# k-xlsx/huff-encoding

Measured on AMD Instinct MI355X. Metric: encode+decode GB/s on 1 GiB bytes at 1/2/4/8 MI355X; % HBM roofline, higher is better.
Workload: dtype u8; 1 GPU; 1 GiB uniform bytes (BASELINE configs[1]), encode+decode, bit-exact; bytes_per_gpu=1073741824, global_bytes=1073741824, compressed_bytes_per_gpu=1073741824, parallelism=shard1

## Files before the change

huff-encoding_amd/csrc/device/hist.hip:

```cpp
#include "bitreader.hpp"

namespace huff::dev {

namespace {

constexpr int kThreads = 256;
constexpr int kCopies = 32;
#ifndef HUFF_HIST_LOGC
#define HUFF_HIST_LOGC 5
#endif


template <int LOGC = 5>
__device__ __forceinline__ void count_word(uint32_t* h, uint32_t w, uint32_t lane_c) {
#pragma unroll
    for (int k = 0; k < 4; ++k) {
        uint32_t b = (w >> (8 * k)) & 0xFFu;
        __hip_atomic_fetch_add(&h[(b << LOGC) | lane_c], 1u, __ATOMIC_RELAXED, __HIP_MEMORY_SCOPE_WORKGROUP);
    }
}

template <int LOGC = 5>
__device__ __forceinline__ void count_masked(uint32_t* h, uint4 v, uint64_t off, uint64_t lo, uint64_t hi,
                                             uint32_t lane_c) {
    uint32_t w[4] = {v.x, v.y, v.z, v.w};
#pragma unroll
    for (int k = 0; k < 16; ++k) {
        uint64_t g = off + k;
        if (g >= lo && g < hi) {
            uint32_t b = (w[k >> 2] >> (8 * (k & 3))) & 0xFFu;
            __hip_atomic_fetch_add(&h[(b << LOGC) | lane_c], 1u, __ATOMIC_RELAXED, __HIP_MEMORY_SCOPE_WORKGROUP);
        }
    }
}

__global__ __launch_bounds__(kThreads) void k_hist(const uint8_t* __restrict__ base, uint64_t lo, uint64_t hi,
                                                   uint32_t nchunks, uint32_t* __restrict__ chunk_hist,
                                                   unsigned long long* __restrict__ gw) {
    __shared__ __attribute__((aligned(16))) uint32_t h[256 * kCopies];
    const uint32_t t = threadIdx.x;
    const uint32_t lane32 = t & 31;
    for (uint32_t i = t; i < 256 * kCopies; i += kThreads) h[i] = 0;
    uint64_t total = 0;
    __syncthreads();

    for (uint32_t c = blockIdx.x; c < nchunks; c += gridDim.x) {
        const uint64_t cbeg = static_cast<uint64_t>(c) * kChunk;
        const bool full = cbeg >= lo && cbeg + kChunk <= hi;
        if (full) {
            const uint4* p = reinterpret_cast<const uint4*>(base + cbeg) + t;
#pragma unroll 1
            for (int r = 0; r < 16; r += 4) {
                uint4 v0 = ld_nt(p + (r + 0) * kThreads);
                uint4 v1 = ld_nt(p + (r + 1) * kThreads);
                uint4 v2 = ld_nt(p + (r + 2) * kThreads);
                uint4 v3 = ld_nt(p + (r + 3) * kThreads);
                count_word(h, v0.x, lane32); count_word(h, v0.y, lane32);
                count_word(h, v0.z, lane32); count_word(h, v0.w, lane32);
                count_word(h, v1.x, lane32); count_word(h, v1.y, lane32);
                count_word(h, v1.z, lane32); count_word(h, v1.w, lane32);
                count_word(h, v2.x, lane32); count_word(h, v2.y, lane32);
                count_word(h, v2.z, lane32); count_word(h, v2.w, lane32);
                count_word(h, v3.x, lane32); count_word(h, v3.y, lane32);
                count_word(h, v3.z, lane32); count_word(h, v3.w, lane32);
            }
        } else {
            for (int r = 0; r < 16; ++r) {
                const uint64_t off = cbeg + static_cast<uint64_t>(r) * kRound + t * 16;
                if (off + 16 <= lo || off >= hi) continue;
                uint4 v;
                if (off + 16 <= hi) {
                    v = *reinterpret_cast<const uint4*>(base + off);
                } else {
                    uint32_t w[4] = {0, 0, 0, 0};
                    for (int k = 0; off + k < hi; ++k) w[k >> 2] |= static_cast<uint32_t>(base[off + k]) << (8 * (k & 3));
                    v = make_uint4(w[0], w[1], w[2], w[3]);
                }
                count_masked(h, v, off, lo, hi, lane32);
            }
        }
        __syncthreads();
        uint32_t s = 0;
#pragma unroll 8
        for (int j = 0; j < kCopies; ++j) {
            uint32_t k = (j + t) & 31;
            s += h[(t << 5) | k];
            h[(t << 5) | k] = 0;
        }
        if (chunk_hist) chunk_hist[static_cast<uint64_t>(c) * 256 + t] = s;
        total += s;
        __syncthreads();
    }
    if (total) atomicAdd(&gw[(blockIdx.x % kHistCopies) * 256 + t], static_cast<unsigned long long>(total));
}

template <int LOGC>
__global__ __launch_bounds__(512) void k_hist1x2(const uint8_t* __restrict__ base, uint64_t lo, uint64_t hi,
                                                 uint32_t nchunks, uint32_t* __restrict__ chunk_hist,
                                                 unsigned long long* __restrict__ gw) {
    constexpr uint32_t C = 1u << LOGC;
    constexpr int T = 256;
    static_assert(LOGC >= 3 && LOGC <= 6, "k_hist1x2 needs 8..64 LDS copies (64 KiB of static LDS at most)");
    static_assert(kChunk / C < 65536, "a copy's 16-bit half counter must not overflow");
    constexpr int NL = kChunk / 16 / T;
    if (blockIdx.x == 0)
        for (uint32_t i = threadIdx.x; i < kHistCopies * 256 + 1; i += 2 * T) gw[i] = 0;
    __shared__ __attribute__((aligned(16))) uint32_t h[256 * C];
    const uint32_t t = threadIdx.x, tl = t & (T - 1), half = t / T;
    const uint32_t lane_c = t & (C - 1);
    const uint32_t inc = half ? 0x10000u : 1u;
    const uint32_t c = 2 * blockIdx.x + half;
    const uint64_t cbeg = static_cast<uint64_t>(c) * kChunk;
    const bool live = c < nchunks;
    const bool full = live && cbeg >= lo && cbeg + kChunk <= hi;
    uint4 v[NL];
    if (full) {
        const uint4* p = reinterpret_cast<const uint4*>(base + cbeg) + tl;
#pragma unroll
        for (int r = 0; r < NL; ++r) v[r] = ld_nt(p + r * T);
    }
    __builtin_amdgcn_sched_barrier(0);
    uint4* h4 = reinterpret_cast<uint4*>(h);
#pragma unroll
    for (uint32_t i = 0; i < 256 * C / 4 / (2 * T); ++i) h4[t + i * 2 * T] = make_uint4(0, 0, 0, 0);
    __builtin_amdgcn_s_waitcnt(0xc07f);
    __builtin_amdgcn_s_barrier();
    auto add = [&](uint32_t w) {
#pragma unroll
        for (int k = 0; k < 4; ++k)
            __hip_atomic_fetch_add(&h[(((w >> (8 * k)) & 0xFFu) << LOGC) | lane_c], inc, __ATOMIC_RELAXED,
                                   __HIP_MEMORY_SCOPE_WORKGROUP);
    };
    if (full) {
#pragma unroll
        for (int r = 0; r < NL; ++r) {
            add(v[r].x);
            add(v[r].y);
            add(v[r].z);
            add(v[r].w);
        }
    } else if (live) {
        for (int r = 0; r < NL; ++r) {
            const uint64_t off = cbeg + static_cast<uint64_t>(r) * (16 * T) + tl * 16;
            if (off + 16 <= lo || off >= hi) continue;
            for (int k = 0; k < 16; ++k)
                if (off + k >= lo && off + k < hi)
                    __hip_atomic_fetch_add(&h[(static_cast<uint32_t>(base[off + k]) << LOGC) | lane_c], inc,
                                           __ATOMIC_RELAXED, __HIP_MEMORY_SCOPE_WORKGROUP);
        }
    }
    __syncthreads();
    if (t < 256) {
        uint32_t s0 = 0, s1 = 0;
#pragma unroll 8
        for (uint32_t j = 0; j < C; ++j) {
            const uint32_t x = h[(t << LOGC) | ((j + t) & (C - 1))];
            s0 += x & 0xFFFFu;
            s1 += x >> 16;
        }
        chunk_hist[static_cast<uint64_t>(2 * blockIdx.x) * 256 + t] = s0;
        if (2 * blockIdx.x + 1 < nchunks) chunk_hist[static_cast<uint64_t>(2 * blockIdx.x + 1) * 256 + t] = s1;
    }
}

__global__ __launch_bounds__(256) void k_rows_sum(const uint32_t* __restrict__ chunk_hist, uint32_t nchunks,
                                                  unsigned long long* __restrict__ gw) {
    const uint32_t t = threadIdx.x;
    uint64_t s0 = 0, s1 = 0, s2 = 0, s3 = 0;
    uint32_t c = blockIdx.x;
    const uint32_t g = gridDim.x;
    for (; c + 3 * g < nchunks; c += 4 * g) {
        s0 += chunk_hist[static_cast<uint64_t>(c) * 256 + t];
        s1 += chunk_hist[static_cast<uint64_t>(c + g) * 256 + t];
        s2 += chunk_hist[static_cast<uint64_t>(c + 2 * g) * 256 + t];
        s3 += chunk_hist[static_cast<uint64_t>(c + 3 * g) * 256 + t];
    }
    for (; c < nchunks; c += g) s0 += chunk_hist[static_cast<uint64_t>(c) * 256 + t];
    const uint64_t s = s0 + s1 + s2 + s3;
    if (s) atomicAdd(&gw[(blockIdx.x % kHistCopies) * 256 + t], static_cast<unsigned long long>(s));
}

#ifndef HUFF_RP_GROUPS
#define HUFF_RP_GROUPS 128
#endif
constexpr uint32_t kRpWaves = 16;
__global__ __launch_bounds__(kRpWaves * 64) void k_rows_publish(const uint32_t* __restrict__ chunk_hist,
                                                                uint32_t nchunks, unsigned long long* gw,
                                                                unsigned long long* host, uint64_t tag) {
    __shared__ uint64_t part[kRpWaves][256];
    __shared__ uint32_t last;
    const uint32_t t = threadIdx.x, lane = t & 63, wave = t >> 6;
    const uint32_t stride = gridDim.x * kRpWaves;
    const uint4* rows = reinterpret_cast<const uint4*>(chunk_hist) + lane;
    uint64_t a0 = 0, a1 = 0, a2 = 0, a3 = 0;
    uint32_t c = blockIdx.x * kRpWaves + wave;
    for (; c + 3 * stride < nchunks; c += 4 * stride) {
        uint4 v[4];
#pragma unroll
        for (int k = 0; k < 4; ++k) v[k] = rows[static_cast<uint64_t>(c + k * stride) * 64];
#pragma unroll
        for (int k = 0; k < 4; ++k) {
            a0 += v[k].x;
            a1 += v[k].y;
            a2 += v[k].z;
            a3 += v[k].w;
        }
    }
    for (; c < nchunks; c += stride) {
        const uint4 v = rows[static_cast<uint64_t>(c) * 64];
        a0 += v.x;
        a1 += v.y;
        a2 += v.z;
        a3 += v.w;
    }
    part[wave][4 * lane] = a0;
    part[wave][4 * lane + 1] = a1;
    part[wave][4 * lane + 2] = a2;
    part[wave][4 * lane + 3] = a3;
    __syncthreads();
    if (t < 256) {
        uint64_t s = 0;
#pragma unroll
        for (uint32_t w = 0; w < kRpWaves; ++w) s += part[w][t];
        if (s)
            __hip_atomic_fetch_add(&gw[(blockIdx.x % kHistCopies) * 256 + t], static_cast<unsigned long long>(s),
                                   __ATOMIC_RELAXED, __HIP_MEMORY_SCOPE_AGENT);
    }
    __syncthreads();
    if (t == 0) {
        const unsigned long long k = __hip_atomic_fetch_add(&gw[kHistCopies * 256], 1ull, __ATOMIC_ACQ_REL,
                                                            __HIP_MEMORY_SCOPE_AGENT);
        last = k == gridDim.x - 1u;
    }
    __syncthreads();
    if (!last || t >= 256) return;
    __atomic_thread_fence(__ATOMIC_ACQUIRE);
    uint64_t tot = 0;
#pragma unroll
    for (uint32_t k = 0; k < kHistCopies; ++k)
        tot += __hip_atomic_load(&gw[k * 256 + t], __ATOMIC_RELAXED, __HIP_MEMORY_SCOPE_AGENT);
    __hip_atomic_store(&host[t], (tag << 48) | tot, __ATOMIC_RELAXED, __HIP_MEMORY_SCOPE_SYSTEM);
}

__global__ __launch_bounds__(256) void k_hist_row(const unsigned long long* __restrict__ gw,
                                                  const uint8_t* __restrict__ in, uint64_t n,
                                                  long long* __restrict__ row) {
    const uint32_t t = threadIdx.x;
    uint64_t tot = 0;
#pragma unroll
    for (uint32_t k = 0; k < kHistCopies; ++k) tot += gw[k * 256 + t];
    row[t] = static_cast<long long>(tot);
    if (t == 0) {
        const uint32_t m = n < 8 ? static_cast<uint32_t>(n) : 8u;
        uint64_t packed = 0;
        for (uint32_t i = 0; i < m; ++i) packed |= static_cast<uint64_t>(in[n - m + i]) << (8 * i);
        row[256] = static_cast<long long>(packed);
        row[257] = m;
    }
}

__global__ __launch_bounds__(256) void k_chunk_bits(const uint32_t* __restrict__ chunk_hist, uint32_t nchunks,
                                                    CodeLens lens, uint64_t* __restrict__ bits) {
    const uint8_t* len = lens.len;
    const uint32_t wave = threadIdx.x >> 6, lane = threadIdx.x & 63;
    const uint32_t c = blockIdx.x * 4 + wave;
    if (c >= nchunks) return;
    uint4 hv = reinterpret_cast<const uint4*>(chunk_hist + static_cast<uint64_t>(c) * 256)[lane];
    uint32_t lv = reinterpret_cast<const uint32_t*>(len)[lane];
    uint64_t s = static_cast<uint64_t>(hv.x) * (lv & 0xFF) + static_cast<uint64_t>(hv.y) * ((lv >> 8) & 0xFF) +
                 static_cast<uint64_t>(hv.z) * ((lv >> 16) & 0xFF) + static_cast<uint64_t>(hv.w) * (lv >> 24);
#pragma unroll
    for (int d = 32; d >= 1; d >>= 1) s += __shfl_down(s, d, 64);
    if (lane == 0) bits[c] = s;
}

__global__ __launch_bounds__(1024) void k_scan_tiles(const uint64_t* __restrict__ bits, uint32_t nchunks,
                                                     uint64_t* __restrict__ start, uint64_t* __restrict__ tsum) {
    __shared__ uint32_t wsum[16];
    const uint32_t t = threadIdx.x, lane = t & 63, wave = t >> 6;
    const uint32_t i = blockIdx.x * 1024 + t;
    const uint32_t v = i < nchunks ? static_cast<uint32_t>(bits[i]) : 0u;
    const uint32_t incl = wave_scan_incl(v);
    if (lane == 63) wsum[wave] = incl;
    __syncthreads();
    uint32_t pre = 0, tot = 0;
#pragma unroll
    for (uint32_t w = 0; w < 16; ++w) {
        pre += (w < wave) ? wsum[w] : 0u;
        tot += wsum[w];
    }
    if (i < nchunks) start[i] = pre + incl - v;
    if (t == 0) tsum[blockIdx.x] = tot;
}

__global__ __launch_bounds__(1024) void k_scan_tsum(uint32_t tiles, uint64_t* __restrict__ tsum) {
    __shared__ uint64_t wsum[16];
    const uint32_t t = threadIdx.x, lane = t & 63, wave = t >> 6;
    const uint32_t per = (tiles + 1023) / 1024;
    const uint32_t lo = t * per < tiles ? t * per : tiles, hi = lo + per < tiles ? lo + per : tiles;
    uint64_t mine = 0;
    for (uint32_t q = lo; q < hi; ++q) mine += tsum[q];
    uint64_t incl = mine;
#pragma unroll
    for (int d = 1; d < 64; d <<= 1) {
        const uint64_t v = __shfl_up(incl, d, 64);
        if (lane >= static_cast<uint32_t>(d)) incl += v;
    }
    if (lane == 63) wsum[wave] = incl;
    __syncthreads();
    uint64_t pre = 0, tot = 0;
#pragma unroll
    for (uint32_t w = 0; w < 16; ++w) {
        pre += (w < wave) ? wsum[w] : 0u;
        tot += wsum[w];
    }
    uint64_t run = pre + incl - mine;
    for (uint32_t q = lo; q < hi; ++q) {
        const uint64_t v = tsum[q];
        tsum[q] = run;
        run += v;
    }
    if (t == 0) tsum[tiles] = tot;
}

__device__ __forceinline__ void publish_total(unsigned long long* host, uint64_t tag, uint64_t total) {
    if (host) __hip_atomic_store(host, (tag << 48) | total, __ATOMIC_RELAXED, __HIP_MEMORY_SCOPE_SYSTEM);
}

__global__ __launch_bounds__(1024) void k_scan_fix_small(uint32_t nchunks, uint64_t base,
                                                         const uint64_t* __restrict__ tsum,
                                                         uint64_t* __restrict__ start,
                                                         unsigned long long* host, uint64_t tag) {
    __shared__ uint64_t off;
    const uint32_t t = threadIdx.x;
    if (t < 64) {
        uint64_t sum = t < blockIdx.x ? tsum[t] : 0;
#pragma unroll
        for (int d = 32; d >= 1; d >>= 1) sum += __shfl_down(sum, d, 64);
        if (t == 0) off = base + sum;
    }
    __syncthreads();
    const uint32_t i = blockIdx.x * 1024 + t;
    if (i < nchunks) start[i] += off;
    if (blockIdx.x == gridDim.x - 1 && t == 0) {
        const uint64_t end = off + tsum[blockIdx.x];
        start[nchunks] = end;
        publish_total(host, tag, end - base);
    }
}

__global__ __launch_bounds__(1024) void k_scan_fix(uint32_t nchunks, uint64_t base, const uint64_t* __restrict__ tsum,
                                                   uint64_t* __restrict__ start, unsigned long long* host,
                                                   uint64_t tag) {
    const uint32_t t = threadIdx.x;
    const uint64_t off = base + tsum[blockIdx.x];
    const uint32_t i = blockIdx.x * 1024 + t;
    if (i < nchunks) start[i] += off;
    if (blockIdx.x == gridDim.x - 1 && t == 0) {
        start[nchunks] = base + tsum[gridDim.x];
        publish_total(host, tag, tsum[gridDim.x]);
    }
}

__global__ __launch_bounds__(256) void k_find_first(const uint8_t* __restrict__ in, uint64_t n,
                                                    const uint8_t* __restrict__ mask,
                                                    unsigned long long* __restrict__ pos) {
    __shared__ uint8_t m[256];
    m[threadIdx.x] = mask[threadIdx.x];
    __syncthreads();
    for (uint64_t i = static_cast<uint64_t>(blockIdx.x) * blockDim.x + threadIdx.x; i < n;
         i += static_cast<uint64_t>(gridDim.x) * blockDim.x) {
        if (m[in[i]]) {
            atomicMin(pos, static_cast<unsigned long long>(i));
            return;
        }
    }
}

}

hipError_t launch_hist(const uint8_t* base, uint64_t lo, uint64_t hi, uint32_t nchunks, uint32_t* chunk_hist,
                       unsigned long long* gw, hipStream_t s, HistDone done) {
    if (nchunks == 0) return hipSuccess;
    if (chunk_hist) {
        launch_k(k_hist1x2<HUFF_HIST_LOGC>, dim3((nchunks + 1) / 2), dim3(512), 0, s, base, lo, hi, nchunks,
                           chunk_hist, gw);
        if (done.host) {
            const uint32_t want = (nchunks + 4 * kRpWaves - 1) / (4 * kRpWaves);
            const uint32_t g = want < HUFF_RP_GROUPS ? want : HUFF_RP_GROUPS;
            launch_k(k_rows_publish, dim3(g), dim3(kRpWaves * 64), 0, s, chunk_hist, nchunks, gw, done.host,
                     done.tag);
            return hipGetLastError();
        }
        const uint32_t g = nchunks < 512 ? nchunks : 512;
        launch_k(k_rows_sum, dim3(g), dim3(256), 0, s, chunk_hist, nchunks, gw);
        return hipGetLastError();
    }
    uint32_t grid = nchunks < 1024 ? nchunks : 1024;
    const hipError_t e = hipMemsetAsync(gw, 0, kHistCopies * 256 * 8, s);
    if (e != hipSuccess) return e;
    launch_k(k_hist, dim3(grid), dim3(kThreads), 0, s, base, lo, hi, nchunks, chunk_hist, gw);
    return hipGetLastError();
}

hipError_t launch_hist_row(const unsigned long long* gw, const uint8_t* in, uint64_t n, long long* row,
                           hipStream_t s) {
    launch_k(k_hist_row, dim3(1), dim3(256), 0, s, gw, in, n, row);
    return hipGetLastError();
}

hipError_t launch_chunk_bits(const uint32_t* chunk_hist, uint32_t nchunks, const CodeLens& len, uint64_t* bits,
                             hipStream_t s) {
    if (nchunks == 0) return hipSuccess;
    launch_k(k_chunk_bits, dim3((nchunks + 3) / 4), dim3(256), 0, s, chunk_hist, nchunks, len, bits);
    return hipGetLastError();
}

hipError_t launch_scan(const uint64_t* bits, uint32_t nchunks, uint64_t base, uint64_t* start, uint64_t* tsum,
                       hipStream_t s, HistDone done) {
    const uint32_t tiles = nchunks ? (nchunks + 1023) / 1024 : 1;
    launch_k(k_scan_tiles, dim3(tiles), dim3(1024), 0, s, bits, nchunks, start, tsum);
    if (tiles <= 64) {
        launch_k(k_scan_fix_small, dim3(tiles), dim3(1024), 0, s, nchunks, base, tsum, start, done.host,
                           done.tag);
    } else {
        launch_k(k_scan_tsum, dim3(1), dim3(1024), 0, s, tiles, tsum);
        launch_k(k_scan_fix, dim3(tiles), dim3(1024), 0, s, nchunks, base, tsum, start, done.host,
                           done.tag);
    }
    return hipGetLastError();
}

hipError_t launch_find_first(const uint8_t* in, uint64_t n, const uint8_t* missing_mask, unsigned long long* pos,
                             hipStream_t s) {
    if (n == 0) return hipSuccess;
    uint64_t blocks = (n + 255) / 256;
    uint32_t grid = blocks < 4096 ? static_cast<uint32_t>(blocks) : 4096;
    launch_k(k_find_first, dim3(grid), dim3(256), 0, s, in, n, missing_mask, pos);
    return hipGetLastError();
}

}
```

huff-encoding_amd/csrc/device/kernels.hpp:

```cpp
#pragma once

#include <hip/hip_runtime.h>
#ifdef __HIPCC__
#include <hip/hip_ext.h>
#endif

#include <cstdint>

namespace huff::dev {

struct LaunchEvents {
    hipEvent_t start = nullptr, stop = nullptr;
};
LaunchEvents& launch_events();
#ifdef __HIPCC__
template <typename F, typename... Args>
inline void launch_k(F kernel, dim3 grid, dim3 block, uint32_t lds, hipStream_t s, Args... args) {
    LaunchEvents& e = launch_events();
    if (e.stop) {
        hipExtLaunchKernelGGL(kernel, grid, block, lds, s, e.start, e.stop, 0, args...);
        e.start = nullptr;
    } else {
        hipLaunchKernelGGL(kernel, grid, block, lds, s, args...);
    }
// ... 333 lines not shown
    const uint8_t* blobs;
    const uint64_t* payload_begin;
    const uint64_t* comp_off;
    const uint32_t* status;
    uint32_t nstreams;
    uint8_t* comp;
    uint64_t comp_cap;
};
struct BatchCountArgs {
    const uint8_t* comp;
    const uint64_t* comp_off;
    const uint64_t* bits;
    const uint64_t* codes;
    const uint32_t* status_in;
    uint32_t nstreams;
    uint64_t* seg;
    uint64_t seg_cap;
    uint64_t* counts;
    uint32_t* status;
};
struct BatchIndexArgs {
    const uint8_t* comp;
    const uint64_t* comp_off;
    const uint64_t* bits;
    const uint64_t* codes;
    const uint64_t* seg;
    uint64_t seg_cap;
    const uint64_t* off;
    const uint64_t* idx_off;
    uint32_t* status;
    uint32_t nstreams;
    uint32_t* sub;
    uint64_t sub_cap;
};
hipError_t launch_batch_blob_offsets(const BatchBlobArgs& a, hipStream_t s);
hipError_t launch_batch_to_bytes(const BatchBlobArgs& a, hipStream_t s);
hipError_t launch_batch_parse(const BatchParseArgs& a, hipStream_t s);
hipError_t launch_batch_unwrap(const BatchUnwrapArgs& a, hipStream_t s);
hipError_t launch_batch_count(const BatchCountArgs& a, hipStream_t s);
hipError_t launch_batch_index(const BatchIndexArgs& a, hipStream_t s);

constexpr uint32_t kDeepWords = 8;
struct DeepPackArgs;
struct DeepSerialArgs {
    const uint8_t* comp;
    uint64_t comp_bytes;
    uint64_t valid_bits;
    const uint32_t* lut;
    uint32_t lut_bits;
    uint8_t* out;
    uint64_t cap;
    unsigned long long* count;
    unsigned long long* end;
};
struct WalkEndArgs {
    const uint8_t* comp;
    uint64_t comp_bytes;
    const uint32_t* lut;
    uint32_t lut_bits;
    const uint64_t* start;
    uint64_t start_v;
    uint32_t start_packed;
    const uint64_t* count;
    uint64_t count_v;
    unsigned long long* end;
};
hipError_t launch_walk_end(const WalkEndArgs& a, hipStream_t s);
hipError_t launch_shift_bits(const uint8_t* src, uint8_t* dst, uint64_t n, uint32_t r, hipStream_t s);
hipError_t launch_pack_deep(const DeepPackArgs& a, hipStream_t s);
hipError_t launch_decode_deep(const DecodeArgs& a, hipStream_t s);
hipError_t launch_decode_deep_serial(const DeepSerialArgs& a, hipStream_t s);

size_t pack_lds_bytes(bool long_codes, uint32_t max_len, uint32_t stage_words);
uint32_t pack_round_bytes();
uint32_t pack_waves_per_group(bool long_codes);
uint32_t pack_groups_per_cu(bool long_codes, uint32_t max_len, size_t lds);
size_t decode_lds_bytes(uint32_t lut_bits);
constexpr uint32_t kDecodeFixed = 10;
constexpr uint32_t kDecodeFixedCheck = 11;

struct HistDone {
    unsigned long long* host = nullptr;
    uint64_t tag = 0;
};
hipError_t launch_hist(const uint8_t* base, uint64_t lo, uint64_t hi, uint32_t nchunks, uint32_t* chunk_hist,
                       unsigned long long* gw, hipStream_t s, HistDone done = HistDone{});
hipError_t launch_hist_row(const unsigned long long* gw, const uint8_t* in, uint64_t n, long long* row,
                           hipStream_t s);
struct alignas(8) CodeLens {
    uint8_t len[256];
};
struct DeepPackArgs {
    CodeLens len;
    const uint32_t* words;
    const uint8_t* in;
    uint64_t n;
    const uint64_t* chunk_start;
    uint32_t nchunks;
    uint8_t* out;
    uint32_t* sub_bit;
};
hipError_t launch_chunk_bits(const uint32_t* chunk_hist, uint32_t nchunks, const CodeLens& len, uint64_t* bits,
                             hipStream_t s);
hipError_t launch_scan(const uint64_t* bits, uint32_t nchunks, uint64_t base, uint64_t* start, uint64_t* tsum,
                       hipStream_t s, HistDone done = HistDone{});
hipError_t launch_pack(bool long_codes, const PackArgs& a, hipStream_t s);
hipError_t launch_decode(const DecodeArgs& a, hipStream_t s);
hipError_t launch_decode_fixed(const DecodeArgs& a, hipStream_t s);
uint32_t decode_fixed_builds();
const char* decode_fixed_build_name(uint32_t i);
uint64_t decode_fixed_build_launches(uint32_t i);
uint32_t decode_fixed_index_forms();
const char* decode_fixed_index_form_name(uint32_t i);
uint64_t decode_fixed_index_form_launches(uint32_t i);
struct RangeReq {
    uint64_t first, count, out_begin, piece0;
    uint32_t index;
    uint32_t pad;
};
struct RangesArgs {
    const uint8_t* comp;
    uint64_t comp_bytes;
    const uint32_t* lut;
    uint32_t lut_bits;
    const uint64_t* chunk_start;
    const uint32_t* sub_bit;
    const uint16_t* sub16;
    const uint64_t* task_base;
    uint32_t nchunks;
    uint64_t n;
    const RangeReq* req;
    uint32_t nreq;
    uint64_t npieces;
    uint8_t* out;
    uint32_t* status;
};
hipError_t launch_decode_ranges(const RangesArgs& a, hipStream_t s);
uint32_t decode_ranges_index_forms();
const char* decode_ranges_index_form_name(uint32_t i);
uint64_t decode_ranges_index_form_launches(uint32_t i);
hipError_t launch_indexless_spec(const IndexlessArgs& a, hipStream_t s);
hipError_t launch_indexless_settle_all(const IndexlessArgs& a, hipStream_t s);
hipError_t launch_indexless_emit(const IndexlessArgs& a, const uint64_t* off, uint8_t* out, hipStream_t s);
hipError_t launch_indexless_counts(const IndexlessArgs& a, hipStream_t s);
constexpr uint32_t mark32_skip(uint32_t m) { return m & 0x3FFu; }
constexpr uint32_t mark32_rel(uint32_t m) { return (m >> 10) & 0x7FFu; }
constexpr uint32_t mark32_seg(uint32_t m, uint32_t base_seg) { return base_seg + (((m >> 21) - base_seg) & 0x7FFu); }
hipError_t launch_indexless_mark_lite(const IndexlessArgs& a, const uint64_t* off, const unsigned long long* woff,
                                      uint64_t* sub_abs, uint64_t sub_cap, hipStream_t st,
                                      uint32_t* mark32 = nullptr, uint32_t* task_seg = nullptr);
constexpr uint64_t kSkipPosMask = (1ull << 48) - 1;
hipError_t launch_indexless_mark(const IndexlessArgs& a, const uint64_t* off, uint64_t* sub_abs, uint32_t shift,
                                 hipStream_t s);
bool indexless_staged(const IndexlessArgs& a);
hipError_t launch_bytemap(const BytemapArgs& a, hipStream_t s);
hipError_t launch_task_sums(const uint8_t* x, uint64_t n, uint64_t* sums, hipStream_t s);
hipError_t launch_task_sums_check(const uint8_t* x, uint64_t n, const uint64_t* sums, unsigned int* err,
                                  hipStream_t s);
hipError_t launch_find_first(const uint8_t* in, uint64_t n, const uint8_t* missing_mask, unsigned long long* pos,
                             hipStream_t s);
hipError_t launch_generate(int kind, uint64_t seed, uint64_t offset, const uint64_t* cdf, uint8_t* out, uint64_t n,
                           hipStream_t s);
hipError_t launch_calib(int mode, const uint8_t* src, uint8_t* dst, uint64_t n, unsigned* sink, uint32_t cu_count,
                        hipStream_t s);

}
```

huff-encoding_amd/csrc/runtime/runtime.cpp:

```cpp
#include "runtime.hpp"

#include "../host/range_plan.hpp"

#include <algorithm>
#include <cctype>
#include <chrono>
#include <cstdio>
#include <cstdlib>
#include <cstring>
#include <string>
#include <thread>

namespace {

std::atomic<uint64_t> g_tree_ids{1};

}

static_assert(huff::kLutPtr == huff::dev::kLutPtr, "host/dectables.hpp mirrors dev::kLutPtr");
static_assert(huff::kLutMaxBits == huff::dev::kLutMaxBits, "host/dectables.hpp mirrors dev::kLutMaxBits");
static_assert(huff::kSsMaxBits == huff::dev::kSsMaxBits, "host/dectables.hpp mirrors dev::kSsMaxBits");
static_assert(huff::kSsSlow == huff::dev::kSsSlow, "host/dectables.hpp mirrors dev::kSsSlow");
static_assert(huff::kLongMaxLen == huff::dev::kLongMaxLen, "host/dectables.hpp mirrors dev::kLongMaxLen");

// ... 176 lines not shown
        return huff::Status::ok();
    }
    hipEvent_t ev[2];
    for (auto& e : ev) {
        if (!free_events.empty()) {
            e = free_events.back();
            free_events.pop_back();
        } else {
            static const unsigned flags = [] {
                const char* f = std::getenv("HUFF_TIME_FENCE");
                if (f && !std::strcmp(f, "none")) return unsigned(hipEventDisableSystemFence);
                if (f && !std::strcmp(f, "device")) return unsigned(hipEventReleaseToDevice);
                return 0u;
            }();
            HIP_TRY(hipEventCreateWithFlags(&e, flags));
        }
    }
    static const bool markers = [] {
        const char* m = std::getenv("HUFF_TIME_MARKERS");
        return m && *m == '1';
    }();
    auto& le = huff::dev::launch_events();
    if (markers) HIP_TRY(hipEventRecord(ev[0], stream));
    else le = {ev[0], ev[1]};
    const hipError_t err = launch();
    const bool none = le.start != nullptr;
    le = {};
    HIP_TRY(err);
    if (none && !markers) HIP_TRY(hipEventRecord(ev[0], stream));
    if (none || markers) HIP_TRY(hipEventRecord(ev[1], stream));
    pending.push_back({name, ev[0], ev[1]});
    return huff::Status::ok();
}

huff::Status huff_ctx::collect_timing() {
    if (pending.empty()) return huff::Status::ok();
    HIP_TRY(hipStreamSynchronize(stream));
    for (auto& p : pending) {
        float ms = 0.f;
        HIP_TRY(hipEventElapsedTime(&ms, p.a, p.b));
        auto& k = kstats[p.name];
        k.first += ms;
        k.second += 1;
        free_events.push_back(p.a);
        free_events.push_back(p.b);
    }
    pending.clear();
    return huff::Status::ok();
}

huff::Status huff_ctx::sync() {
    HIP_TRY(hipStreamSynchronize(stream));
    return huff::Status::ok();
}

huff::Status huff_ctx::upload_dec_tables(const huff_tree* t, const huff::DecTables** dt, bool for_decode) {
    HUFF_TRY(t->dec_tables(dt));
    if (lut_tree_id == t->id) return huff::Status::ok();
    if (for_decode && (*dt)->all8 && !huff::fixed8_disabled()) return huff::Status::ok();
    const size_t bytes = (*dt)->lut.size() * 4;
    HUFF_TRY(pin_lut.ensure(bytes));
    std::memcpy(pin_lut.p, (*dt)->lut.data(), bytes);
    HUFF_TRY(d_lut.ensure(bytes));
    HIP_TRY(hipStreamWaitEvent(copy_stream, lut_free, 0));
    HIP_TRY(hipMemcpyAsync(d_lut.p, pin_lut.p, bytes, hipMemcpyHostToDevice, copy_stream));
    HIP_TRY(hipEventRecord(pin_lut.ev, copy_stream));
    HIP_TRY(hipStreamWaitEvent(stream, pin_lut.ev, 0));
    lut_tree_id = t->id;
    return huff::Status::ok();
}

huff::Status huff_enc::init(huff_ctx* c, const uint8_t* d, uint64_t nbytes) {
    if (reinterpret_cast<uintptr_t>(d) & 15)
        return huff::Status::err(HUFF_E_INVALID_ARG, "device input must be 16-byte aligned");
    if (nbytes >= (1ull << 48))
        return huff::Status::err(HUFF_E_INVALID_ARG, "one job holds fewer than 2^48 bytes");
    ctx = c;
    d_in = d;
    n = nbytes;
    nchunks = static_cast<uint32_t>((n + huff::dev::kChunk - 1) / huff::dev::kChunk);
    have_hist = packed = sums_valid = false;
    const size_t nc = std::max<uint32_t>(nchunks, 1);
    HUFF_TRY(chunk_hist.ensure(nc * 256 * 4));
    HUFF_TRY(gw.ensure(huff::dev::kHistCopies * 256 * 8 + 8));

    HUFF_TRY(chunk_bits.ensure(nc * 8));
    HUFF_TRY(chunk_start.ensure((nc + 1) * 8));
    HUFF_TRY(tsum.ensure((nc / 1024 + 2) * 8));
    HUFF_TRY(sub_bit.ensure(((n + huff::dev::kIdx - 1) / huff::dev::kIdx + 1) * 4));
    HUFF_TRY(mask.ensure(256));
    HUFF_TRY(pos.ensure(8));
    return huff::Status::ok();
}

class SpinWait {
public:
    bool check_due() {
        if ((++spin_ & 255) != 0) return false;
        const auto now = std::chrono::steady_clock::now();
        if (now - t0_ < std::chrono::milliseconds(2)) return false;
        std::this_thread::yield();
        if (now - last_ < std::chrono::milliseconds(1)) return false;
        last_ = now;
        return true;
    }

private:
    std::chrono::steady_clock::time_point t0_ = std::chrono::steady_clock::now(), last_{};
    uint64_t spin_ = 0;
};

huff::Status TaggedWords::arm(size_t words, huff::dev::HistDone* done) {
    HUFF_TRY(pin.ensure(words * 8));
    if (!dev) {
        std::memset(pin.p, 0, words * 8);
        HIP_TRY(hipHostGetDevicePointer(&dev, pin.p, 0));
    }
    seq = (seq % 0xFFFF) + 1;
    done->host = static_cast<unsigned long long*>(dev);
    done->tag = seq;
    return huff::Status::ok();
}

huff::Status TaggedWords::wait(hipStream_t s, uint64_t tag, uint64_t* out, size_t words, const char* what) {
    const uint64_t* hw = static_cast<const uint64_t*>(pin.p);
    size_t b = 0;
    SpinWait sw;
    while (b < words) {
        const uint64_t v = __atomic_load_n(&hw[b], __ATOMIC_ACQUIRE);
        if ((v >> 48) == tag) {
            out[b++] = v & ((1ull << 48) - 1);
            continue;
        }
        if (sw.check_due()) {
            const hipError_t q = hipStreamQuery(s);
            if (q == hipSuccess && (__atomic_load_n(&hw[b], __ATOMIC_ACQUIRE) >> 48) != tag)
                return huff::Status::err(HUFF_E_HIP, what);
            if (q != hipSuccess && q != hipErrorNotReady) HIP_TRY(q);
        }
    }
    return huff::Status::ok();
}

huff::Status huff_enc::launch_publish(uint64_t* tag) {
    huff::dev::HistDone done;
    HUFF_TRY(ctx->weights.arm(256, &done));
    HUFF_TRY(ctx->timed("hist", [&] {
        return huff::dev::launch_hist(d_in, 0, n, nchunks, static_cast<uint32_t*>(chunk_hist.p),
                                      static_cast<unsigned long long*>(gw.p), ctx->stream, done);
    }));
    *tag = done.tag;
    return huff::Status::ok();
}

static huff::Status pending_guard(const huff_ctx* ctx, const huff_enc* e) {
    if (ctx->hist_pending && ctx->hist_pending != e)
        return huff::Status::err(HUFF_E_STATE, "another job's pass 1 is pending on this context (huff_enc_hist_launch): "
                                               "compress or hist that job first");
    return huff::Status::ok();
}

huff::Status huff_enc::hist_launch() {
    HUFF_TRY(ctx->activate());
    HUFF_TRY(pending_guard(ctx, this));
    if (nchunks == 0 || ctx->hist_pending == this) return huff::Status::ok();
    uint64_t tag = 0;
    HUFF_TRY(launch_publish(&tag));
    ctx->hist_pending = this;
    ctx->hist_pending_tag = tag;
    return huff::Status::ok();
}

huff::Status huff_enc::hist() {
    HUFF_TRY(ctx->activate());
    HUFF_TRY(pending_guard(ctx, this));
    if (nchunks == 0) {
        for (int b = 0; b < 256; ++b) w[b] = 0;
        have_hist = true;
        packed = false;
        return huff::Status::ok();
    }
    uint64_t tag = 0;
    if (ctx->hist_pending == this) {
        tag = ctx->hist_pending_tag;
        ctx->hist_pending = nullptr;
    } else {
        HUFF_TRY(launch_publish(&tag));
    }
    HUFF_TRY(ctx->weights.wait(ctx->stream, tag, w, 256, "pass 1 finished without publishing its weights"));
    have_hist = true;
    packed = false;
    return huff::Status::ok();
}

huff::Status huff_enc::hist_known(const uint64_t counts[256]) {
    HUFF_TRY(ctx->activate());
    if (ctx->hist_pending == this) ctx->hist_pending = nullptr;
    std::memcpy(w, counts, sizeof w);
    have_hist = true;
    packed = false;
    if (nchunks == 0) return huff::Status::ok();
    return ctx->timed("hist", [&] {
        return huff::dev::launch_hist(d_in, 0, n, nchunks, static_cast<uint32_t*>(chunk_hist.p),
                                      static_cast<unsigned long long*>(gw.p), ctx->stream);
    });
}

huff::Status huff_enc::hist_row(long long* d_row) {
    HUFF_TRY(ctx->activate());
    if (ctx->hist_pending == this) ctx->hist_pending = nullptr;
    hipStream_t s = ctx->stream;
    have_hist = false;
    if (nchunks == 0) {
        HIP_TRY(hipMemsetAsync(d_row, 0, 258 * 8, s));
        return huff::Status::ok();
    }
    HUFF_TRY(ctx->timed("hist", [&] {
        hipError_t e = huff::dev::launch_hist(d_in, 0, n, nchunks, static_cast<uint32_t*>(chunk_hist.p),
                                              static_cast<unsigned long long*>(gw.p), s);
        if (e != hipSuccess) return e;
        return huff::dev::launch_hist_row(static_cast<const unsigned long long*>(gw.p), d_in, n, d_row, s);
    }));
    return huff::Status::ok();
}

huff::Status huff_enc::bits(const huff_tree* t, uint64_t* total) {
    if (!have_hist) return huff::Status::err(HUFF_E_STATE, "huff_enc_hist must run before bits/pack");
    const huff::EncTables& et = t->enc_tables();
    uint64_t b = 0;
    for (int i = 0; i < 256; ++i) {
        if (w[i] && et.len[i] == 0) {
            uint8_t m[256];
            for (int k = 0; k < 256; ++k) m[k] = (w[k] && et.len[k] == 0) ? 1 : 0;
            HUFF_TRY(ctx->activate());
            HIP_TRY(hipMemcpy(mask.p, m, 256, hipMemcpyHostToDevice));
            unsigned long long init = ~0ull;
            HIP_TRY(hipMemcpy(pos.p, &init, 8, hipMemcpyHostToDevice));
            HIP_TRY(huff::dev::launch_find_first(d_in, n, static_cast<const uint8_t*>(mask.p),
                                                 static_cast<unsigned long long*>(pos.p), ctx->stream));
            unsigned long long p = 0;
            HIP_TRY(hipMemcpyAsync(&p, pos.p, 8, hipMemcpyDeviceToHost, ctx->stream));
            HUFF_TRY(ctx->sync());
            uint8_t letter = 0;
            HIP_TRY(hipMemcpy(&letter, d_in + p, 1, hipMemcpyDeviceToHost));
            huff::Status st = huff::Status::err(HUFF_E_MISSING_LETTER, "letter not found in codes");
            st.missing_letter = letter;
            return st;
        }
        b += w[i] * et.len[i];
    }
    *total = b;
    return huff::Status::ok();
}

huff::Status huff_enc::check_sums(const uint8_t* d_out) {
    if (!sums_valid || !huff::decode_check_mode()) return huff::Status::ok();
    HUFF_TRY(ctx->d_err.ensure(32));
    unsigned int* err = static_cast<unsigned int*>(ctx->d_err.p);
    const unsigned int init[2] = {0u, ~0u};
    HIP_TRY(hipMemcpyAsync(err, init, 8, hipMemcpyHostToDevice, ctx->stream));
    HIP_TRY(huff::dev::launch_task_sums_check(d_out, n, static_cast<const uint64_t*>(task_sums.p), err, ctx->stream));
    unsigned int e[2] = {};
    HIP_TRY(hipMemcpyAsync(e, err, 8, hipMemcpyDeviceToHost, ctx->stream));
    HUFF_TRY(ctx->sync());
    if (e[0] == 0) return huff::Status::ok();
    return huff::Status::err(HUFF_E_CORRUPT, "decode self-check: letter checksums differ in " + std::to_string(e[0]) +
                                                 " task(s) of 4096 letters; first: task " + std::to_string(e[1]));
}

huff::PackStamps& huff::pack_stamps() {
    static thread_local PackStamps p;
    return p;
}

huff::Status huff_enc::pack(const huff_tree* t, uint64_t base, const uint8_t* prev_tail, size_t prev_tail_len,
                            uint8_t* d_out, size_t out_cap, uint64_t* total) {
    auto& ps = huff::pack_stamps();
    ps.bits = ps.launch = ps.launched = {};
    uint64_t tb = 0;
    HUFF_TRY(bits(t, &tb));
    ps.bits = std::chrono::steady_clock::now();
    compact_index = false;
    const uint64_t need = ((base & 7) + tb + 7) / 8;
    if (total) *total = tb;
    if (need > out_cap) return huff::Status::err(HUFF_E_BUFFER_TOO_SMALL, "output buffer too small");
    if (prev_tail_len > 8) return huff::Status::err(HUFF_E_INVALID_ARG, "prev_tail holds at most 8 bytes");
    HUFF_TRY(ctx->activate());
    hipStream_t s = ctx->stream;
    sums_valid = false;
    if (huff::decode_check_mode() && n) {
        HUFF_TRY(task_sums.ensure(((n + huff::dev::kTaskSym - 1) / huff::dev::kTaskSym) * 8));
        HIP_TRY(huff::dev::launch_task_sums(d_in, n, static_cast<uint64_t*>(task_sums.p), s));
        sums_valid = true;
    }
    const huff::EncTables& et = t->enc_tables();
    const bool long_codes = et.maxlen > huff::dev::kShortMaxLen;
    if ((base & 7) == 0 && et.maxlen == 8 && !huff::fixed8_disabled()) {
        bool all8 = true;
        for (int b = 0; b < 256; ++b) all8 &= (w[b] == 0 || et.len[b] == 8);
        if (all8) {
            huff::dev::BytemapArgs m{};
            m.src = d_in;
            m.dst = d_out;
            m.n = n;
            for (int b = 0; b < 256; ++b) m.map[b] = static_cast<uint8_t>(et.code[b]);
            m.nchunks = nchunks;
// ... 785 lines not shown
```

huff-encoding_amd/csrc/runtime/runtime.hpp:

```cpp
#pragma once

#include <hip/hip_runtime.h>

#include <atomic>
#include <chrono>
#include <functional>
#include <map>
#include <memory>
#include <mutex>
#include <string>
#include <vector>

#include "../device/kernels.hpp"
#include "../host/dectables.hpp"
#include "../host/huff_coding.hpp"

namespace huff {

inline Status hip_status(hipError_t e, const char* what) {
    if (e == hipSuccess) return Status::ok();
    return Status::err(HUFF_E_HIP, std::string(what) + ": " + hipGetErrorString(e));
}
#define HIP_TRY_RT(expr) HUFF_TRY(::huff::hip_status((expr), #expr))

// ... 76 lines not shown
namespace huff {
struct IndexlessSync;
struct FileWs;
}

struct huff_wenc;

struct huff_ctx {
    int device = 0;
    int cu_count = 256;
    hipStream_t own = nullptr;
    hipStream_t stream = nullptr;
    hipStream_t copy_stream = nullptr;
    hipEvent_t lut_free = nullptr;
    TaggedWords weights;
    const huff_enc* hist_pending = nullptr;
    uint64_t hist_pending_tag = 0;
    TaggedWords total;
    PinnedBuf pin_lut;
    DevBuf d_in, d_out;
    DevBuf d_lut;
    const uint16_t* lut_u16(uint32_t off) const {
        return reinterpret_cast<const uint16_t*>(static_cast<const uint32_t*>(d_lut.p) + off);
    }
    DevBuf d_align;
    DevBuf d_comp_align;
    DevBuf d_err;
    std::shared_ptr<huff::IndexlessSync> idx_ws;
    DevBuf idx_sub_abs;
    DevBuf idx_mark32, idx_task_seg;
    huff::IndexlessSync& indexless_ws();
    std::shared_ptr<huff::FileWs> file_ws;
    std::shared_ptr<huff_wenc> wdec_ws;
    uint64_t lut_tree_id = 0;

    struct Timed {
        std::string name;
        hipEvent_t a, b;
    };
    bool timing = false;
    std::vector<Timed> pending;
    std::vector<hipEvent_t> free_events;
    std::map<std::string, std::pair<double, uint64_t>> kstats;
    huff::Status timed(const char* name, const std::function<hipError_t()>& launch);
    huff::Status collect_timing();

    huff::Status activate() const;
    huff::Status upload_dec_tables(const huff_tree* t, const huff::DecTables** dt, bool for_decode = false);
    huff::Status sync();
};

struct huff_enc {
    huff_ctx* ctx = nullptr;
    const uint8_t* d_in = nullptr;
    uint64_t n = 0;
    uint32_t nchunks = 0;
    DevBuf chunk_hist, gw, chunk_bits, chunk_start, tsum, sub_bit, mask, pos;
    DevBuf deep_words;
    DevBuf task_base, sub16;
    bool compact_index = false;
    DevBuf task_sums;
    bool sums_valid = false;
    huff::Status check_sums(const uint8_t* d_out);
    huff::Status expand_index();
    uint64_t w[256] = {};
    bool have_hist = false;
    bool packed = false;
    uint64_t packed_tree_id = 0;
    uint8_t packed_len[256] = {};
    uint64_t packed_code[256] = {};
    std::vector<uint32_t> packed_deep;
    bool packed_any_tree = false;
    void remember_tree(const huff_tree* t);
    bool codes_match(const huff_tree* t) const;
    uint64_t bit_base = 0, total_bits = 0;
    bool index_pending = false;
    huff::Status ensure_index();
    void set_packed(const huff_tree* t, uint64_t base, uint64_t bits, bool pending, bool compact);

    huff::Status init(huff_ctx* c, const uint8_t* d, uint64_t nbytes);
    huff::Status hist();
    huff::Status hist_launch();
    huff::Status launch_publish(uint64_t* tag);
    huff::Status hist_known(const uint64_t counts[256]);
    huff::Status hist_row(long long* d_row);
    huff::Status bits(const huff_tree* t, uint64_t* total);
    huff::Status pack(const huff_tree* t, uint64_t bit_base, const uint8_t* prev_tail, size_t prev_tail_len,
                      uint8_t* d_out, size_t out_cap, uint64_t* total);
    huff::Status decode(const huff_tree* t, const uint8_t* d_comp, uint64_t comp_bytes, uint8_t* d_out);
    DevBuf range_req, range_status;
    huff::Status decode_ranges(const huff_tree* t, const uint8_t* d_comp, uint64_t comp_bytes, const uint64_t* first,
                               const uint64_t* count, const uint64_t* out_begin, uint32_t nreq, uint8_t* d_out,
                               size_t out_cap, uint32_t* status);
    huff::Status download_index(huff_index_host& idx);
    huff::Status upload_index(const huff_index_host& idx);
};

namespace huff {
Status weights_from_host(huff_ctx* ctx, const uint8_t* bytes, size_t n, ByteWeights& out);
Status weights_threaded_from_host(huff_ctx* ctx, const uint8_t* bytes, size_t n, size_t thread_num,
                                  ByteWeights& out);
Status compress_host(huff_ctx* ctx, const uint8_t* bytes, size_t n, const huff_tree* t, huff_compress_data** out);
Status decompress_host(huff_ctx* ctx, const huff_compress_data* cd, uint8_t* out, size_t cap, size_t* out_len);
Status decompress_range_host(huff_ctx* ctx, const huff_compress_data* cd, uint64_t first, uint64_t count,
                             uint8_t* out, size_t cap);
Status file_compress(huff_ctx* ctx, const char* src, const char* dst, size_t block_size);
Status file_decompress(huff_ctx* ctx, const char* src, const char* dst, size_t block_size);
Status parse_block_size(const char* s, size_t* out);
Status run_checked_decode(huff_ctx* ctx, dev::DecodeArgs& a, const std::function<hipError_t()>& launch);
Status decode_indexless_dev(huff_ctx* ctx, const uint8_t* d_comp, uint64_t comp_bytes, uint64_t valid_bits,
                            const huff_tree* t, DevBuf& out, uint64_t* nsym, uint8_t* d_user = nullptr,
                            size_t user_cap = 0, unsigned long long* d_end = nullptr);
struct IndexlessSync {
    const DecTables* dt = nullptr;
    DevBuf s, x0, c, off, flag, tsum, samp, tm, dl, fixlist, chain, rec;
    DevBuf wtot, woff;
    dev::IndexlessArgs a{};
    uint64_t total = 0;
    bool block_off = false;
};
Status indexless_sync(huff_ctx* ctx, const uint8_t* d_comp, uint64_t comp_bytes, uint64_t valid_bits,
                      const huff_tree* t, IndexlessSync& st, bool need_off = true,
                      const std::function<Status()>& before_wait = nullptr);
Status indexless_mark(huff_ctx* ctx, IndexlessSync& st, DevBuf& sub_abs, uint32_t shift = 8);
Status decode_indexless_host(huff_ctx* ctx, const uint8_t* comp, size_t len, uint64_t valid_bits,
                             const huff_tree* t, std::vector<uint8_t>& out);
}
```

Before: 1243 GB/s.

## Fuse histogram row reduction and publish into the pass-1 histogram kernel

```diff
diff --git a/huff-encoding_amd/csrc/device/hist.hip b/huff-encoding_amd/csrc/device/hist.hip
--- a/huff-encoding_amd/csrc/device/hist.hip
+++ b/huff-encoding_amd/csrc/device/hist.hip
@@ -97,14 +97,12 @@
 template <int LOGC>
 __global__ __launch_bounds__(512) void k_hist1x2(const uint8_t* __restrict__ base, uint64_t lo, uint64_t hi,
                                                  uint32_t nchunks, uint32_t* __restrict__ chunk_hist,
-                                                 unsigned long long* __restrict__ gw) {
+                                                 unsigned long long* bins, uint32_t parts, HistDone done) {
     constexpr uint32_t C = 1u << LOGC;
     constexpr int T = 256;
     static_assert(LOGC >= 3 && LOGC <= 6, "k_hist1x2 needs 8..64 LDS copies (64 KiB of static LDS at most)");
     static_assert(kChunk / C < 65536, "a copy's 16-bit half counter must not overflow");
     constexpr int NL = kChunk / 16 / T;
-    if (blockIdx.x == 0)
-        for (uint32_t i = threadIdx.x; i < kHistCopies * 256 + 1; i += 2 * T) gw[i] = 0;
     __shared__ __attribute__((aligned(16))) uint32_t h[256 * C];
     const uint32_t t = threadIdx.x, tl = t & (T - 1), half = t / T;
     const uint32_t lane_c = t & (C - 1);
@@ -150,6 +148,7 @@
         }
     }
     __syncthreads();
+    const bool publish = done.host || done.row;
     if (t < 256) {
         uint32_t s0 = 0, s1 = 0;
 #pragma unroll 8
@@ -160,102 +159,38 @@
         }
         chunk_hist[static_cast<uint64_t>(2 * blockIdx.x) * 256 + t] = s0;
         if (2 * blockIdx.x + 1 < nchunks) chunk_hist[static_cast<uint64_t>(2 * blockIdx.x + 1) * 256 + t] = s1;
-    }
-}
-
-__global__ __launch_bounds__(256) void k_rows_sum(const uint32_t* __restrict__ chunk_hist, uint32_t nchunks,
-                                                  unsigned long long* __restrict__ gw) {
-    const uint32_t t = threadIdx.x;
-    uint64_t s0 = 0, s1 = 0, s2 = 0, s3 = 0;
-    uint32_t c = blockIdx.x;
-    const uint32_t g = gridDim.x;
-    for (; c + 3 * g < nchunks; c += 4 * g) {
-        s0 += chunk_hist[static_cast<uint64_t>(c) * 256 + t];
-        s1 += chunk_hist[static_cast<uint64_t>(c + g) * 256 + t];
-        s2 += chunk_hist[static_cast<uint64_t>(c + 2 * g) * 256 + t];
-        s3 += chunk_hist[static_cast<uint64_t>(c + 3 * g) * 256 + t];
-    }
-    for (; c < nchunks; c += g) s0 += chunk_hist[static_cast<uint64_t>(c) * 256 + t];
-    const uint64_t s = s0 + s1 + s2 + s3;
-    if (s) atomicAdd(&gw[(blockIdx.x % kHistCopies) * 256 + t], static_cast<unsigned long long>(s));
-}
-
-#ifndef HUFF_RP_GROUPS
-#define HUFF_RP_GROUPS 128
-#endif
-constexpr uint32_t kRpWaves = 16;
-__global__ __launch_bounds__(kRpWaves * 64) void k_rows_publish(const uint32_t* __restrict__ chunk_hist,
-                                                                uint32_t nchunks, unsigned long long* gw,
-                                                                unsigned long long* host, uint64_t tag) {
-    __shared__ uint64_t part[kRpWaves][256];
-    __shared__ uint32_t last;
-    const uint32_t t = threadIdx.x, lane = t & 63, wave = t >> 6;
-    const uint32_t stride = gridDim.x * kRpWaves;
-    const uint4* rows = reinterpret_cast<const uint4*>(chunk_hist) + lane;
-    uint64_t a0 = 0, a1 = 0, a2 = 0, a3 = 0;
-    uint32_t c = blockIdx.x * kRpWaves + wave;
-    for (; c + 3 * stride < nchunks; c += 4 * stride) {
-        uint4 v[4];
-#pragma unroll
-        for (int k = 0; k < 4; ++k) v[k] = rows[static_cast<uint64_t>(c + k * stride) * 64];
-#pragma unroll
-        for (int k = 0; k < 4; ++k) {
-            a0 += v[k].x;
-            a1 += v[k].y;
-            a2 += v[k].z;
-            a3 += v[k].w;
-        }
-    }
-    for (; c < nchunks; c += stride) {
-        const uint4 v = rows[static_cast<uint64_t>(c) * 64];
-        a0 += v.x;
-        a1 += v.y;
-        a2 += v.z;
-        a3 += v.w;
-    }
-    part[wave][4 * lane] = a0;
-    part[wave][4 * lane + 1] = a1;
-    part[wave][4 * lane + 2] = a2;
-    part[wave][4 * lane + 3] = a3;
-    __syncthreads();
-    if (t < 256) {
-        uint64_t s = 0;
-#pragma unroll
-        for (uint32_t w = 0; w < kRpWaves; ++w) s += part[w][t];
-        if (s)
-            __hip_atomic_fetch_add(&gw[(blockIdx.x % kHistCopies) * 256 + t], static_cast<unsigned long long>(s),
-                                   __ATOMIC_RELAXED, __HIP_MEMORY_SCOPE_AGENT);
-    }
-    __syncthreads();
-    if (t == 0) {
-        const unsigned long long k = __hip_atomic_fetch_add(&gw[kHistCopies * 256], 1ull, __ATOMIC_ACQ_REL,
+        if (publish) {
+            constexpr uint64_t kSum = (1ull << kHistCntShift) - 1;
+            const uint32_t p = blockIdx.x % parts;
+            const uint32_t adders = (gridDim.x - p + parts - 1) / parts;
+            unsigned long long* word = bins + 256 + p * 256 + t;
+            const uint32_t s = s0 + s1;
+            const uint64_t was = __hip_atomic_fetch_add(word, (1ull << kHistCntShift) | s, __ATOMIC_RELAXED,
+                                                        __HIP_MEMORY_SCOPE_AGENT);
+            if ((was >> kHistCntShift) + 1 == adders) {
+                __hip_atomic_store(word, 0ull, __ATOMIC_RELAXED, __HIP_MEMORY_SCOPE_AGENT);
+                const uint64_t rowsum = (was & kSum) + s;
+                const uint64_t bin = __hip_atomic_fetch_add(&bins[t], (1ull << 48) | rowsum, __ATOMIC_RELAXED,
                                                             __HIP_MEMORY_SCOPE_AGENT);
-        last = k == gridDim.x - 1u;
-    }
-    __syncthreads();
-    if (!last || t >= 256) return;
-    __atomic_thread_fence(__ATOMIC_ACQUIRE);
-    uint64_t tot = 0;
-#pragma unroll
-    for (uint32_t k = 0; k < kHistCopies; ++k)
-        tot += __hip_atomic_load(&gw[k * 256 + t], __ATOMIC_RELAXED, __HIP_MEMORY_SCOPE_AGENT);
-    __hip_atomic_store(&host[t], (tag << 48) | tot, __ATOMIC_RELAXED, __HIP_MEMORY_SCOPE_SYSTEM);
-}
-
-__global__ __launch_bounds__(256) void k_hist_row(const unsigned long long* __restrict__ gw,
-                                                  const uint8_t* __restrict__ in, uint64_t n,
-                                                  long long* __restrict__ row) {
-    const uint32_t t = threadIdx.x;
-    uint64_t tot = 0;
-#pragma unroll
-    for (uint32_t k = 0; k < kHistCopies; ++k) tot += gw[k * 256 + t];
-    row[t] = static_cast<long long>(tot);
-    if (t == 0) {
-        const uint32_t m = n < 8 ? static_cast<uint32_t>(n) : 8u;
-        uint64_t packed = 0;
-        for (uint32_t i = 0; i < m; ++i) packed |= static_cast<uint64_t>(in[n - m + i]) << (8 * i);
-        row[256] = static_cast<long long>(packed);
-        row[257] = m;
+                if ((bin >> 48) + 1 == parts) {
+                    __hip_atomic_store(&bins[t], 0ull, __ATOMIC_RELAXED, __HIP_MEMORY_SCOPE_AGENT);
+                    const uint64_t total = (bin & ((1ull << 48) - 1)) + rowsum;
+                    if (done.host)
+                        __hip_atomic_store(&done.host[t], (done.tag << 48) | total, __ATOMIC_RELAXED,
+                                           __HIP_MEMORY_SCOPE_SYSTEM);
+                    else
+                        done.row[t] = static_cast<long long>(total);
+                }
+            }
+            if (done.row && blockIdx.x == 0 && t == 0) {
+                const uint64_t n = hi - lo;
+                const uint32_t m = n < 8 ? static_cast<uint32_t>(n) : 8u;
+                uint64_t packed = 0;
+                for (uint32_t i = 0; i < m; ++i) packed |= static_cast<uint64_t>(base[hi - m + i]) << (8 * i);
+                done.row[256] = static_cast<long long>(packed);
+                done.row[257] = m;
+            }
+        }
     }
 }
 
@@ -380,32 +315,18 @@
 }
 
 hipError_t launch_hist(const uint8_t* base, uint64_t lo, uint64_t hi, uint32_t nchunks, uint32_t* chunk_hist,
-                       unsigned long long* gw, hipStream_t s, HistDone done) {
+                       void* gw, hipStream_t s, HistDone done) {
     if (nchunks == 0) return hipSuccess;
     if (chunk_hist) {
         launch_k(k_hist1x2<HUFF_HIST_LOGC>, dim3((nchunks + 1) / 2), dim3(512), 0, s, base, lo, hi, nchunks,
-                           chunk_hist, gw);
-        if (done.host) {
-            const uint32_t want = (nchunks + 4 * kRpWaves - 1) / (4 * kRpWaves);
-            const uint32_t g = want < HUFF_RP_GROUPS ? want : HUFF_RP_GROUPS;
-            launch_k(k_rows_publish, dim3(g), dim3(kRpWaves * 64), 0, s, chunk_hist, nchunks, gw, done.host,
-                     done.tag);
-            return hipGetLastError();
-        }
-        const uint32_t g = nchunks < 512 ? nchunks : 512;
-        launch_k(k_rows_sum, dim3(g), dim3(256), 0, s, chunk_hist, nchunks, gw);
+                 chunk_hist, static_cast<unsigned long long*>(gw), hist_parts(nchunks), done);
         return hipGetLastError();
     }
     uint32_t grid = nchunks < 1024 ? nchunks : 1024;
     const hipError_t e = hipMemsetAsync(gw, 0, kHistCopies * 256 * 8, s);
     if (e != hipSuccess) return e;
-    launch_k(k_hist, dim3(grid), dim3(kThreads), 0, s, base, lo, hi, nchunks, chunk_hist, gw);
-    return hipGetLastError();
-}
-
-hipError_t launch_hist_row(const unsigned long long* gw, const uint8_t* in, uint64_t n, long long* row,
-                           hipStream_t s) {
-    launch_k(k_hist_row, dim3(1), dim3(256), 0, s, gw, in, n, row);
+    launch_k(k_hist, dim3(grid), dim3(kThreads), 0, s, base, lo, hi, nchunks, chunk_hist,
+             static_cast<unsigned long long*>(gw));
     return hipGetLastError();
 }
 
diff --git a/huff-encoding_amd/csrc/device/kernels.hpp b/huff-encoding_amd/csrc/device/kernels.hpp
--- a/huff-encoding_amd/csrc/device/kernels.hpp
+++ b/huff-encoding_amd/csrc/device/kernels.hpp
@@ -439,11 +439,22 @@
 struct HistDone {
     unsigned long long* host = nullptr;
     uint64_t tag = 0;
-};
+    long long* row = nullptr;
+};
+constexpr uint32_t kHistParts = 64;
+constexpr uint32_t kHistCntShift = 40;
+constexpr uint64_t kHistMaxAdders = (1u << 23) - 1;
+inline uint32_t hist_parts(uint32_t nchunks) {
+    const uint64_t groups = (static_cast<uint64_t>(nchunks) + 1) / 2;
+    const uint64_t need = (groups + kHistMaxAdders - 1) / kHistMaxAdders;
+    const uint64_t want = need > kHistParts ? need : kHistParts;
+    return static_cast<uint32_t>(want < groups ? want : groups);
+}
+inline size_t hist_totals_bytes(uint32_t nchunks) {
+    return (256 + static_cast<size_t>(hist_parts(nchunks)) * 256) * 8;
+}
 hipError_t launch_hist(const uint8_t* base, uint64_t lo, uint64_t hi, uint32_t nchunks, uint32_t* chunk_hist,
-                       unsigned long long* gw, hipStream_t s, HistDone done = HistDone{});
-hipError_t launch_hist_row(const unsigned long long* gw, const uint8_t* in, uint64_t n, long long* row,
-                           hipStream_t s);
+                       void* gw, hipStream_t s, HistDone done = HistDone{});
 struct alignas(8) CodeLens {
     uint8_t len[256];
 };
diff --git a/huff-encoding_amd/csrc/runtime/runtime.cpp b/huff-encoding_amd/csrc/runtime/runtime.cpp
--- a/huff-encoding_amd/csrc/runtime/runtime.cpp
+++ b/huff-encoding_amd/csrc/runtime/runtime.cpp
@@ -282,7 +282,9 @@
     have_hist = packed = sums_valid = false;
     const size_t nc = std::max<uint32_t>(nchunks, 1);
     HUFF_TRY(chunk_hist.ensure(nc * 256 * 4));
-    HUFF_TRY(gw.ensure(huff::dev::kHistCopies * 256 * 8 + 8));
+    const void* gw_was = gw.p;
+    HUFF_TRY(gw.ensure(huff::dev::hist_totals_bytes(nchunks)));
+    if (gw.p != gw_was) gw_zero = false;
 
     HUFF_TRY(chunk_bits.ensure(nc * 8));
     HUFF_TRY(chunk_start.ensure((nc + 1) * 8));
@@ -342,13 +344,21 @@
     return huff::Status::ok();
 }
 
+huff::Status huff_enc::launch_pass1(const huff::dev::HistDone& done) {
+    const bool totals = done.host || done.row;
+    if (totals && !gw_zero) HIP_TRY(hipMemsetAsync(gw.p, 0, gw.cap, ctx->stream));
+    const huff::Status st = ctx->timed("hist", [&] {
+        return huff::dev::launch_hist(d_in, 0, n, nchunks, static_cast<uint32_t*>(chunk_hist.p), gw.p, ctx->stream,
+                                      done);
+    });
+    if (totals) gw_zero = !st;
+    return st;
+}
+
 huff::Status huff_enc::launch_publish(uint64_t* tag) {
     huff::dev::HistDone done;
     HUFF_TRY(ctx->weights.arm(256, &done));
-    HUFF_TRY(ctx->timed("hist", [&] {
-        return huff::dev::launch_hist(d_in, 0, n, nchunks, static_cast<uint32_t*>(chunk_hist.p),
-                                      static_cast<unsigned long long*>(gw.p), ctx->stream, done);
-    }));
+    HUFF_TRY(launch_pass1(done));
     *tag = done.tag;
     return huff::Status::ok();
 }
@@ -387,7 +397,12 @@
     } else {
         HUFF_TRY(launch_publish(&tag));
     }
-    HUFF_TRY(ctx->weights.wait(ctx->stream, tag, w, 256, "pass 1 finished without publishing its weights"));
+    const huff::Status st =
+        ctx->weights.wait(ctx->stream, tag, w, 256, "pass 1 finished without publishing its weights");
+    if (st) {
+        gw_zero = false;
+        return st;
+    }
     have_hist = true;
     packed = false;
     return huff::Status::ok();
@@ -400,10 +415,7 @@
     have_hist = true;
     packed = false;
     if (nchunks == 0) return huff::Status::ok();
-    return ctx->timed("hist", [&] {
-        return huff::dev::launch_hist(d_in, 0, n, nchunks, static_cast<uint32_t*>(chunk_hist.p),
-                                      static_cast<unsigned long long*>(gw.p), ctx->stream);
-    });
+    return launch_pass1(huff::dev::HistDone{});
 }
 
 huff::Status huff_enc::hist_row(long long* d_row) {
@@ -415,13 +427,9 @@
         HIP_TRY(hipMemsetAsync(d_row, 0, 258 * 8, s));
         return huff::Status::ok();
     }
-    HUFF_TRY(ctx->timed("hist", [&] {
-        hipError_t e = huff::dev::launch_hist(d_in, 0, n, nchunks, static_cast<uint32_t*>(chunk_hist.p),
-                                              static_cast<unsigned long long*>(gw.p), s);
-        if (e != hipSuccess) return e;
-        return huff::dev::launch_hist_row(static_cast<const unsigned long long*>(gw.p), d_in, n, d_row, s);
-    }));
-    return huff::Status::ok();
+    huff::dev::HistDone done;
+    done.row = d_row;
+    return launch_pass1(done);
 }
 
 huff::Status huff_enc::bits(const huff_tree* t, uint64_t* total) {
diff --git a/huff-encoding_amd/csrc/runtime/runtime.hpp b/huff-encoding_amd/csrc/runtime/runtime.hpp
--- a/huff-encoding_amd/csrc/runtime/runtime.hpp
+++ b/huff-encoding_amd/csrc/runtime/runtime.hpp
@@ -182,6 +182,8 @@
     huff::Status hist();
     huff::Status hist_launch();
     huff::Status launch_publish(uint64_t* tag);
+    huff::Status launch_pass1(const huff::dev::HistDone& done);
+    bool gw_zero = false;
     huff::Status hist_known(const uint64_t counts[256]);
     huff::Status hist_row(long long* d_row);
     huff::Status bits(const huff_tree* t, uint64_t* total);
diff --git a/profiles/pass1_single_launch/summarize.py b/profiles/pass1_single_launch/summarize.py
--- /dev/null
+++ b/profiles/pass1_single_launch/summarize.py
@@ -0,0 +1,16 @@
+import glob
+import json
+import os
+import statistics as st
+import sys
+
+d = os.path.join(os.path.dirname(os.path.abspath(__file__)), sys.argv[1])
+runs = {}
+for f in sorted(glob.glob(os.path.join(d, "*.json"))):
+    size, build = os.path.basename(f)[:-5].rsplit("_", 1)[0].split("_", 1)
+    r = json.loads(open(f).read().strip().splitlines()[-1])
+    runs.setdefault((size, build), []).append((r["ms_per_step"], r["kernels"]["hist"]["avg_ms"], r["value"]))
+for (size, build), v in sorted(runs.items()):
+    ms, hist, val = zip(*v)
+    print(f"{size:5} {build:18} ms_per_step median {st.median(ms):.4f} min {min(ms):.4f} max {max(ms):.4f} | "
+          f"hist ms median {st.median(hist):.5f} | GB/s median {st.median(val):.1f}  ({len(v)} runs)")
```

New measurement: 1235 GB/s. No clear change (-0.6%).
